# JohannesBuchner/UltraNest

Measured on AMD Instinct MI355X. Metric: proposal-points filtered/sec (MLFriends.inside) + region-rebuild ms, N=4000 d=50, higher is better.
Workload: dtype f64; 1 GPU; C5: N=4000 live points, d=50, P=1e6 proposals/step/GPU drawn uniformly inside the wrapping ellipsoid (set E), AffineLayer, 30 bootstraps; one step = MLFriends.inside on a batch resident in HBM; the timed loop visits 3 distinct batches in turn; n_live=4000, d=50, bootstraps=30, parallelism=proposal rows sharded over 1 GPU(s), region replicated

## Files before the change

include/mlfriends_hip.h:

```cpp
#ifndef MLFRIENDS_HIP_H
#define MLFRIENDS_HIP_H

#include <stddef.h>
#include <stdint.h>

#ifdef __cplusplus
extern "C" {
#endif

#define MLF_ABI_VERSION 5

#define MLF_E_BADARG 1
#define MLF_E_DIM 2
#define MLF_E_NODEVICE 3
#define MLF_E_STATE 4

#define MLF_MAX_DIM 1024

int mlf_abi_version(void);
const char *mlf_last_error(void);
int mlf_device_count(int *count);
int mlf_set_device(int device);
int mlf_device_name(char *buf, size_t buflen);
int mlf_synchronize(void);
// ... 254 lines not shown
                           uint64_t seed, uint64_t offset, int slots_per_poll, mlf_usermodel *model, double *out_u,
                           double *out_p, double *out_L, int64_t *out_start, double *out_tleft, double *out_tright,
                           int32_t *out_taken, int32_t *out_taken_it, int32_t *out_iters, double *out_widths,
                           double *counts, uint64_t *next_offset);

int mlf_region_time_inside_dev(mlf_region *r, const double *d_pts, size_t np, uint8_t *d_mask,
                               void *stream, int reps, float *ms_total, float *ms_scan);

int mlf_region_inside_dev_timed(mlf_region *r, const double *d_pts, size_t np, uint8_t *d_mask,
                                void *stream);
int mlf_region_timing_collect(mlf_region *r, int *ncalls, double *ms_prep, double *ms_scan,
                              double *ms_rest);
int mlf_region_timing_filter_launches(mlf_region *r, int *nlaunches, double *ms_total);
int mlf_region_timing_filter_launch_ms(mlf_region *r, double *ms, int cap, int *nlaunches);
int mlf_region_filter_info(mlf_region *r, size_t np, int *active, int *kdim, int *ntiles32);
int mlf_comm_unique_id(char *id_out, size_t len );
int mlf_comm_init_rank(const char *id, size_t len, int nranks, int rank);
int mlf_comm_init(int ndev);
int mlf_allreduce_max(double *values, size_t count);
int mlf_comm_destroy(void);

int mlf_region_debug_stats(mlf_region *r, unsigned long long *out, int cap);
int mlf_region_debug_fused_stamps(mlf_region *r, int block, unsigned long long *out, int cap);
int mlf_bench_fp64_valu(double *tflops);

#ifdef __cplusplus
}
#endif
#endif
```

ultranest_amd/_lib.py:

```python
import ctypes
import os

import numpy as np

_HERE = os.path.dirname(os.path.abspath(__file__))
LIB_PATH = os.path.join(_HERE, "libmlfriends_hip.so")

ABI_VERSION = 5

_c_double_p = ctypes.c_void_p
_sz = ctypes.c_size_t
_dbl = ctypes.c_double
_int = ctypes.c_int
_vp = ctypes.c_void_p

SIGNATURES = {
    "mlf_abi_version": [],
    "mlf_last_error": [],
    "mlf_device_count": [_vp],
    "mlf_set_device": [_int],
    "mlf_device_name": [_vp, _sz],
    "mlf_synchronize": [],
    "mlf_set_option": [ctypes.c_char_p, ctypes.c_longlong],
    "mlf_get_option": [ctypes.c_char_p, _vp],
# ... 68 lines not shown
    "mlf_walkers_update_live": [_vp, _vp, _sz, _vp, _vp],
    "mlf_walkers_step_dev": [_vp, _dbl, _dbl, _int, _dbl, ctypes.c_uint64, ctypes.c_uint64, _int, _dbl, _dbl, _int, _vp, _dbl,
                             _vp, _vp],
    "mlf_walkers_step_graph": [_vp, _dbl, _dbl, _int, _dbl, ctypes.c_uint64, ctypes.c_uint64, _int, _dbl, _dbl, _int, _vp, _dbl,
                               _vp, _vp],
    "mlf_walkers_rounds_dev": [_vp, _dbl, _dbl, _int, _dbl, ctypes.c_uint64, ctypes.c_uint64, _int, _dbl, _dbl, _int, _vp, _dbl,
                               _int, _vp, _vp, _vp, _vp],
    "mlf_walkers_export": [_vp, _vp, _vp, _vp, _vp, _vp, _vp, _vp, _vp, _vp],
    "mlf_host_changed_rows": [_vp, _vp, _sz, _sz, _vp, _sz, _vp],
    "mlf_host_draw_selection": [_vp, _vp, _sz, _sz, _vp],
    "mlf_counter_create": [_vp, _sz, _sz, _vp, _int, _int],
    "mlf_counter_destroy": [_vp],
    "mlf_counter_reset": [_vp],
    "mlf_counter_passing_node": [_vp, ctypes.c_int64, _dbl, _sz, _vp, _vp, _vp, _sz, _vp, _vp],
    "mlf_counter_state": [_vp, _vp, _vp, _vp, _vp, _vp, _vp, _sz, _vp],
    "mlf_region_inside_dev_timed": [_vp, _vp, _sz, _vp, _vp],
    "mlf_region_timing_collect": [_vp, _vp, _vp, _vp, _vp],
    "mlf_region_timing_filter_launches": [_vp, _vp, _vp],
    "mlf_region_timing_filter_launch_ms": [_vp, _vp, ctypes.c_int, _vp],
    "mlf_region_filter_info": [_vp, _sz, _vp, _vp, _vp],
    "mlf_bench_fp64_valu": [_vp],
    "mlf_region_debug_stats": [_vp, _vp, _int],
    "mlf_region_debug_fused_stamps": [_vp, _int, _vp, _int],
    "mlf_comm_unique_id": [_vp, _sz],
    "mlf_comm_init_rank": [_vp, _sz, _int, _int],
    "mlf_comm_init": [_int],
    "mlf_allreduce_max": [_vp, _sz],
    "mlf_comm_destroy": [],
    "mlf_usermodel_compile": [ctypes.c_char_p, ctypes.c_char_p, _int, _vp, _sz, _vp, _vp, _sz],
    "mlf_usermodel_create": [_vp, _sz, _sz, _int, _vp, _sz, _vp],
    "mlf_usermodel_destroy": [_vp],
    "mlf_usermodel_eval": [_vp, _vp, _sz, _vp, _vp],
    "mlf_usermodel_eval_dev": [_vp, _vp, _sz, _vp, _vp, _vp, _vp],
    "mlf_region_refill_user": [_vp, _int, _sz, ctypes.c_uint64, ctypes.c_uint64, _dbl, _vp, _vp, _vp, _vp, _sz, _vp, _vp, _vp],
    "mlf_region_set_tregion": [_vp, _vp, _vp, _vp, _dbl],
    "mlf_region_set_tregion_center": [_vp, _vp],
    "mlf_region_clear_tregion": [_vp],
    "mlf_region_set_tregion_wide": [_vp, _sz, _vp, _vp, _vp, _dbl],
    "mlf_usermodel_compile_variant": [ctypes.c_char_p, ctypes.c_char_p, _int, _int, _vp, _sz, _vp, _vp, _sz],
    "mlf_usermodel_compile_sums": [ctypes.c_char_p, ctypes.c_char_p, _int, _int, _int, _vp, _sz, _vp, _vp, _sz],
    "mlf_usermodel_create_variant": [_vp, _sz, _sz, _int, _int, _vp, _sz, _vp],
    "mlf_usermodel_create_sum": [_vp, _sz, _sz, _int, _int, _sz, _vp, _sz, _vp],
    "mlf_usermodel_create_derived": [_vp, _sz, _sz, _sz, _vp, _sz, _vp],
    "mlf_usermodel_derive": [_vp, _vp, _sz, _vp],
    "mlf_usermodel_derive_dev": [_vp, _vp, _sz, _vp, _vp],
    "mlf_usermodel_derive_lds_bytes": [_sz, _sz],
# ... 146 lines not shown
```

ultranest_amd/csrc/mlf_debug.hip:

```cpp
#include <hip/hip_runtime.h>

#include <atomic>
#include <vector>

#include "../../include/mlfriends_hip.h"
#include "mlf_host.hpp"
#include "mlf_sample.hpp"

using namespace mlf;

extern "C" {

int mlf_debug_forget_grants(unsigned long long *grants_so_far) {
  if (grants_so_far) *grants_so_far = g_grant_calls.load(std::memory_order_relaxed);
  g_grant_epoch.fetch_add(1u, std::memory_order_acq_rel);
  return 0;
}

int mlf_debug_philox(uint64_t seed, unsigned stream, size_t nblocks, uint32_t *out) {
  if (!out) return fail_arg(MLF_E_BADARG, "null pointer");
  if (nblocks == 0) return 0;
  if (int rc = ensure_ctx()) return rc;
  Ctx &c = g_ctx;
  CK(c.out.reserve(nblocks * 4 * sizeof(unsigned)));
// ... 73 lines not shown
  *nlaunches = n;
  return 0;
}

int mlf_region_filter_info(mlf_region *r, size_t np, int *active, int *kdim, int *ntiles32) {
  if (!r || !active || !kdim || !ntiles32) return fail_arg(MLF_E_BADARG, "null pointer");
  *active = (r->ready && r->use_scan && plan_batch(r->filter, r, BATCH_INSIDE, (long long)np, r->r2).filter) ? 1 : 0;
  *kdim = r->filter.ks * 16;
  *ntiles32 = r->filter.ntiles32;
  return 0;
}

int mlf_region_debug_fused_stamps(mlf_region *r, int block, unsigned long long *out, int cap) {
  if (!r) return fail_arg(MLF_E_BADARG, "null region");
  FilterCtx &f = r->filter;
  if (out && cap > 0) {
    for (int i = 0; i < cap; ++i) out[i] = 0ull;
    if (f.fstamps.p && f.stamp_block >= 0) {
      CK(hipStreamSynchronize(g_ctx.stream));
      CK(hipMemcpy(out, f.fstamps.p, (size_t)(cap < 16 ? cap : 16) * sizeof(unsigned long long), hipMemcpyDeviceToHost));
    }
  }
  f.stamp_block = block;
  return 0;
}

int mlf_region_debug_stats(mlf_region *r, unsigned long long *out, int cap) {
  if (!r || !out || cap < 6) return fail_arg(MLF_E_BADARG, "bad argument");
  FilterCtx &f = r->filter;
  for (int i = 0; i < cap; ++i) out[i] = 0;
  CK(hipDeviceSynchronize());
  if (f.misc.p) {
    unsigned m[8];
    CK(hipMemcpy(m, f.misc.p, sizeof m, hipMemcpyDeviceToHost));
    out[0] = m[4];
  }
  if (f.segcnt.p && f.segcnt.cap >= sizeof(unsigned)) {
    const size_t n = (size_t)f.last.nsegs;
    std::vector<unsigned> c(n);
    if (n) CK(hipMemcpy(c.data(), f.segcnt.p, n * sizeof(unsigned), hipMemcpyDeviceToHost));
    unsigned long long sum = 0, mx = 0;
    for (unsigned v : c) {
      sum += v;
      mx = v > mx ? v : mx;
    }
    out[2] = sum;
// ... 83 lines not shown
```

ultranest_amd/csrc/mlf_filter.hpp:

```cpp
#pragma once
#include "mlf_common.hpp"
#include "mlf_prep4.hpp"

#define MLF_FILTER_MAXD 128

constexpr int kFilterMaxSplit = 16;

namespace mlf {

struct FilterArgs {
  const void *refF;
  const void *qF;
  const float *tlo, *thi;
  int ntiles32;
  long long ngroups;
  long long nq;
  int *best;
  unsigned long long *list;
  unsigned seg_cap;
  unsigned *seg_count;
  unsigned *counters;
  int tile0, tile1;
  const int *qmap;
  const unsigned *ngroups_dev;
// ... 88 lines not shown
};
#define MLF_FOR_EACH_DP_MID(X)                                                                \
  X(2) X(4) X(6) X(8) X(10) X(12) X(14) X(16) X(18) X(20) X(22) X(24) X(26) X(28) X(30) X(32) \
  X(36) X(40) X(44) X(48) X(50) X(52) X(56)
bool mid_usable(int dp);
int mid_range_quads(long long ngroups, int ntiles32);
hipError_t launch_inside_mid(const MidArgs &a, int ny, hipStream_t s);

struct FusedArgs {
  Prep4Args p;
  const void *refF;
  int ntiles32;
  int tile0, tile1;
  void *cq;
  float *ctlo, *cthi;
  int *cmap, *cmin;
  unsigned *ccount;
  unsigned ccap;
  unsigned long long *stamps;
  unsigned stamp_block;
  unsigned variant;
};
bool fused_usable(int dp);
hipError_t launch_prep_sweep(const FusedArgs &a, hipStream_t s, int waves = 8);

void launch_phase_finish(void *cq, float *ctlo, float *cthi, int *cmap, unsigned *ccount, unsigned *ngroups_dst,
                         int ks, hipStream_t s);

struct RecheckArgs {
  const unsigned long long *list;
  unsigned seg_cap;
  const unsigned *seg_count;
  const double *refR;
  int n, d, dp;
  const double *q;
  long long ldq, ldk, nq;
  double r2;
  int *best;
};

void launch_ref_stats(const double *refR, int n, int d, int dp, double *stats, double *scratch, hipStream_t s,
                      unsigned long long *keys = nullptr);
void launch_quant_refs(const double *refR, int n, int npad32, int d, int dp, int ks,
                       const double *stats, void *refF, hipStream_t s, void *refFm = nullptr, const int *perm = nullptr,
                       double *rows_out = nullptr, int nrows_out = 0);
void launch_ref_rank(const unsigned long long *keys, int n, int *perm, hipStream_t s);
void launch_quant_queries(const double *q, long long ldq, long long nq, long long nqpad, int d_src, int d, int ks,
// ... 16 lines not shown
```

ultranest_amd/csrc/mlf_fused.hip:

```cpp
#include "mlf_filter.hpp"
#include "mlf_dpp_dev.hpp"
#include "mlf_filter_dev.hpp"
#include "mlf_prep4.hpp"

#include <math.h>

namespace mlf {

typedef float float16v __attribute__((ext_vector_type(16)));
typedef _Float16 half2v __attribute__((ext_vector_type(2)));
typedef _Float16 half8v __attribute__((ext_vector_type(8)));
typedef float float2v __attribute__((ext_vector_type(2)));
typedef unsigned uint4v __attribute__((ext_vector_type(4)));

#ifndef MLF_OPERAND_STEPS
#define MLF_OPERAND_STEPS 4
#endif
namespace {

template <int DP, int NW = 8>
struct F4 {
  static constexpr int NS = (DP + 15) / 16;
  static constexpr int KS = (DP + 6 + 15) / 16;
  static constexpr int NT = (KS + 1) / 2;
  static constexpr int NE = (DP + 31) / 32;
  static constexpr int KMIN = DP <= 32 ? DP - 1 : (DP == 50 ? 49 : DP - 3);
  static constexpr int NLT = NS + (NE > 1 ? NS - 2 : 0);
  static constexpr int NPC = (DP + 3) / 4;
  static constexpr size_t r16(size_t x) { return (x + 15) / 16 * 16; }
  static constexpr size_t WAVE = NW == 8 ? r16((size_t)NPC * 1024 + 512) : r16((size_t)32 * DP * 8);
  static constexpr size_t FRAG = (size_t)(2 * NT * NS + 2 * NLT) * 1024 + (size_t)(32 * NE + 32 * NT) * 4 + (size_t)(16 * NS) * 8;
  static constexpr size_t LDS = r16(FRAG) + NW * WAVE + 64 + (NW == 8 ? 0 : 128);
};

template <int NS, int NE, int NT>
struct F4Steps {
  static constexpr int NYE = NS + (NE > 1 ? NS - 2 : 0);
  static constexpr int N = NYE + NT * NS;
  static constexpr int ye_find(int i, bool want_t) {
    int c = 0;
    for (int s = 0; s < NS; ++s)
      for (int t = 0; t < NE; ++t)
        if (s >= 2 * t) {
          if (c == i) return want_t ? t : s;
          ++c;
        }
    return 0;
  }
  static constexpr bool is_t(int i) { return i >= NYE; }
  static constexpr int tile(int i) { return i < NYE ? ye_find(i, true) : (i - NYE) % NT; }
  static constexpr int kstep(int i) { return i < NYE ? ye_find(i, false) : (i - NYE) / NT; }
  static constexpr int fragment(int i) { return i < NYE ? (tile(i) ? NS : 0) + kstep(i) - 2 * tile(i) : tile(i) * NS + kstep(i); }
  static constexpr bool first_of_chain(int i) { return i >= NYE && kstep(i) == 0; }
};

// ... 9 lines not shown
__device__ __forceinline__ float half_sum(float v) { return half_sum32(v); }
__device__ __forceinline__ int min3i(int a, int b, int c) {
  const int m = a < b ? a : b;
  return m < c ? m : c;
}
constexpr int kPosInf = 0x7f800000;
__device__ __forceinline__ int tree_min(const float16v &c, int run) {
  const int m0 = min3i(__float_as_int(c[0]), __float_as_int(c[1]), __float_as_int(c[2]));
  const int m1 = min3i(__float_as_int(c[3]), __float_as_int(c[4]), __float_as_int(c[5]));
  const int m2 = min3i(__float_as_int(c[6]), __float_as_int(c[7]), __float_as_int(c[8]));
  const int m3 = min3i(__float_as_int(c[9]), __float_as_int(c[10]), __float_as_int(c[11]));
  const int m4 = min3i(__float_as_int(c[12]), __float_as_int(c[13]), __float_as_int(c[14]));
  return min3i(min3i(m0, m1, m2), min3i(m3, m4, __float_as_int(c[15])), run);
}
template <int I, int NM, int NV>
__device__ __forceinline__ void pin_step() {
  if constexpr (I < NM) {
    __builtin_amdgcn_sched_group_barrier(0x008, 1, 0);
    __builtin_amdgcn_sched_group_barrier(0x002, (NV * (I + 1)) / NM - (NV * I) / NM, 0);
    pin_step<I + 1, NM, NV>();
  }
}

}

template <int DP, int NW, bool SQ>
__global__ __launch_bounds__(64 * NW, NW == 8 ? 1 : 2) void k_prep_sweep(FusedArgs a) {
  using C = F4<DP, NW>;
  constexpr int NS = C::NS, NT = C::NT, NE = C::NE, KS = C::KS, QW = 4;
  extern __shared__ __attribute__((aligned(16))) unsigned char ldsf[];
  const uint4 *Th = reinterpret_cast<const uint4 *>(ldsf);
  const uint4 *Tl = Th + NT * NS * 64;
  const uint4 *Lh = Tl + NT * NS * 64;
  const uint4 *Ll = Lh + C::NLT * 64;
  float *y0l = reinterpret_cast<float *>(const_cast<uint4 *>(Ll + C::NLT * 64));
  float *csl = y0l + 32 * NE;
  double *ctrl = reinterpret_cast<double *>(csl + 32 * NT);
  const int tid = threadIdx.x, lane = tid & 63;
  const int wv = __builtin_amdgcn_readfirstlane(tid >> 6);
  const int p32 = lane & 31, h = lane >> 5;
  unsigned char *area = ldsf + C::r16(C::FRAG) + (size_t)wv * C::WAVE;
  double *xs = reinterpret_cast<double *>(area);
  const int d = a.p.d;
  constexpr float up = 1.0f + 0x1p-18f, dn = 1.0f - 0x1p-18f;
  unsigned *wg_keep = reinterpret_cast<unsigned *>(ldsf + C::r16(C::FRAG) + NW * C::WAVE);
  unsigned &wg_base = wg_keep[8];
  const bool stamp_on = a.stamps != nullptr && blockIdx.x == a.stamp_block && wv == 0;
  auto stamp = [&](int k) __attribute__((always_inline)) {
    if (stamp_on) {
      const unsigned long long t = __builtin_readcyclecounter();
      if (lane == 0) a.stamps[k] = t;
    }
  };
  stamp(0);

  const double sigma = a.p.stats[0];
  const bool sig_ok = sigma >= 0x1p-60 && sigma <= 0x1p60;
  const float sig_f = sig_ok ? (float)sigma : 1.0f;
  if (blockIdx.x == 0 && tid == 0 && a.p.counters) {
    a.p.counters[0] = 0;
    a.p.counters[1] = 0;
  }
  if (!(a.variant & 1u)) {
    uint4 *dst = reinterpret_cast<uint4 *>(ldsf);
    const uint4 *srcT = reinterpret_cast<const uint4 *>(a.p.TtF);
    const uint4 *srcL = reinterpret_cast<const uint4 *>(a.p.LtF);
    for (int e = tid; e < 2 * NT * NS * 64; e += 64 * NW) dst[e] = srcT[e];
    if constexpr (!SQ)
      for (int e = tid; e < 2 * C::NLT * 64; e += 64 * NW) dst[2 * NT * NS * 64 + e] = srcL[e];
  } else {
    typedef __attribute__((address_space(1))) const void gp_t;
    typedef __attribute__((address_space(3))) void lp_t;
    constexpr int NPT = 2 * NT * NS, NPL = SQ ? 0 : 2 * C::NLT;
    const unsigned char *srcT = reinterpret_cast<const unsigned char *>(a.p.TtF);
    const unsigned char *srcL = reinterpret_cast<const unsigned char *>(a.p.LtF);
#pragma unroll
    for (int i = 0; i < (NPT + NPL + NW - 1) / NW; ++i) {
      const int pc = wv + NW * i;
      if (pc < NPT)
        __builtin_amdgcn_global_load_lds((gp_t *)(srcT + (size_t)pc * 1024 + lane * 16), (lp_t *)(ldsf + (size_t)pc * 1024), 16, 0, 0);
      else if (pc < NPT + NPL)
        __builtin_amdgcn_global_load_lds((gp_t *)(srcL + (size_t)(pc - NPT) * 1024 + lane * 16), (lp_t *)(ldsf + (size_t)pc * 1024), 16, 0, 0);
    }
  }
  static_assert(32 * NE <= 64 * NW && 32 * NT <= 64 * NW && 16 * NS <= 64 * NW, "one thread per constant");
  if constexpr (!SQ)
    if (tid < 32 * NE) y0l[tid] = a.p.y0[tid];
  if (tid < 32 * NT) {
    const int col = f4_column(tid >> 5, tid & 31);
    csl[tid] = col < DP ? 2.0f * (float)(sigma * a.p.stats[8 + col]) : 0.0f;
  }
  if (tid < 16 * NS) ctrl[tid] = tid < d ? (double)a.p.c.s_x * a.p.lay_ctr[tid] : 0.0;

  const long long np = a.p.np;
  const long long ngroups = (np + 31) / 32;
  const long long set = (long long)blockIdx.x * NW + wv;
  const long long g0 = set * QW;
  const long long total = np * (long long)d;
  typedef __attribute__((address_space(1))) const void gptr_t;
  typedef __attribute__((address_space(3))) void lptr_t;
  const int units = 16 * d, nfull = units >> 6, rem = units & 63;
  auto fetch_group = [&](long long grp) __attribute__((always_inline)) {
    if (grp >= ngroups) return;
    const long long base = grp * 32 * (long long)d;
    if (base + 32 * (long long)d <= total) {
      const unsigned char *src = reinterpret_cast<const unsigned char *>(a.p.pts + base) + lane * 16;
      int nf = nfull;
      asm volatile("" : "+s"(nf));
#pragma unroll
      for (int ib = 0; ib < C::NPC; ib += 4) {
        gptr_t *gp = (gptr_t *)(src + ib * 1024);
        lptr_t *lp = (lptr_t *)(area + ib * 1024);
        if (ib < nf) __builtin_amdgcn_global_load_lds(gp, lp, 16, 0, 0);
        if (ib + 1 < C::NPC && ib + 1 < nf) __builtin_amdgcn_global_load_lds(gp, lp, 16, 1024, 0);
        if (ib + 2 < C::NPC && ib + 2 < nf) __builtin_amdgcn_global_load_lds(gp, lp, 16, 2048, 0);
        if (ib + 3 < C::NPC && ib + 3 < nf) __builtin_amdgcn_global_load_lds(gp, lp, 16, 3072, 0);
      }
      if (lane < rem)
        __builtin_amdgcn_global_load_lds((gptr_t *)(src + nf * 1024), (lptr_t *)(area + nf * 1024), 16, 0, 0);
    } else {
#pragma nounroll
      for (int e = lane; e < units; e += 64) {
        const long long g = base + 2 * e;
        double v0 = 0.0, v1 = 0.0;
        if (g < total) v0 = a.p.pts[g];
        if (g + 1 < total) v1 = a.p.pts[g + 1];
        xs[2 * e] = v0;
        xs[2 * e + 1] = v1;
      }
    }
  };
  fetch_group(g0);
  if (a.variant & 1u) asm volatile("s_waitcnt vmcnt(0)" ::: "memory");
  __syncthreads();
  stamp(1);

  const float sqrt_k = __builtin_sqrtf((float)(16 * KS));
  const float namax = (float)a.p.stats[1] * up;
  float cs2 = 0.0f;
  for (int e = 0; e < 32 * NT; ++e) cs2 = __builtin_fmaf(csl[e], csl[e], cs2);
  const float csn = 0.5f * __builtin_sqrtf(cs2) * up;
  const float zeta_scale = sig_f * a.p.c.zt * up;
  const float zeta0 = (a.p.c.g_chain * csn + sig_f * a.p.c.zt_abs) * up + 0x1p-100f;
  const float kappa = -2.0f * sig_f * a.p.c.inv_st_sx;
  const double sr = sigma * sqrt(a.p.r2);
  const float sr_lo = (float)(sr * (1.0 - 0x1p-30)) * dn;
  const float sr_hi = (float)(sr * (1.0 + 0x1p-30)) * up;
  const float inv_sx2 = a.p.c.inv_sx * a.p.c.inv_sx, inv_slsx2 = a.p.c.inv_sl_sx * a.p.c.inv_sl_sx;
  const double sxd = (double)a.p.c.s_x;

  half8v bq[QW][KS];
  float tlo[QW], thi[QW];
  half8v hia[NS], loa[NS];
  float dn2a = 0.0f;
  typedef __attribute__((address_space(3))) const double lds_cdouble;
  lds_cdouble *xrow = (lds_cdouble *)(xs + p32 * d + 8 * h);
  lds_cdouble *crow = (lds_cdouble *)(ctrl + 8 * h);
  asm volatile("" : "+v"(xrow), "+v"(crow));
  auto operands = [&]() __attribute__((always_inline)) {
    float dn2 = 0.0f;
    constexpr int SB = MLF_OPERAND_STEPS;
#pragma unroll
    for (int sb = 0; sb < NS; sb += SB) {
      double xv[SB][8], cv[SB][8];
#pragma unroll
      for (int s = sb; s < sb + SB && s < NS; ++s)
#pragma unroll
        for (int jj = 0; jj < 8; ++jj) {
          if (16 * s + (jj & ~1) >= DP) continue;
          xv[s - sb][jj] = xrow[16 * s + jj];
// ... 27 lines not shown
          }
          float x32[2];
#pragma unroll
          for (int e = 0; e < 2; ++e) {
            const int jj = 2 * j2 + e;
            const int k = 16 * s + 8 * h + jj;
            const bool ok = 16 * s + 8 + jj < C::KMIN || k < d;
            const double x = __builtin_fma(xv[s - sb][jj], sxd, -cv[s - sb][jj]);
            x32[e] = ok ? (float)x : 0.0f;
            dn2 = __builtin_fmaf(x32[e], x32[e], dn2);
          }
          const half2v hp = __builtin_convertvector((float2v){x32[0], x32[1]}, half2v);
          const float2v res = {x32[0] - (float)hp[0], x32[1] - (float)hp[1]};
          const half2v lp = __builtin_convertvector(res, half2v);
          hia[s][2 * j2] = hp[0];
          hia[s][2 * j2 + 1] = hp[1];
          loa[s][2 * j2] = lp[0];
          loa[s][2 * j2 + 1] = lp[1];
        }
      }
    }
    return dn2;
  };
  auto frag = [&](const uint4 *base, int idx) __attribute__((always_inline)) {
    union { uint4 u; half8v h8; } cv;
    cv.u = base[idx * 64 + lane];
    return cv.h8;
  };
  if (g0 < ngroups) {
    asm volatile("s_waitcnt vmcnt(0)" ::: "memory");
    __builtin_amdgcn_wave_barrier();
    stamp(2);
    dn2a = operands();
    asm volatile("s_waitcnt lgkmcnt(0)" ::: "memory");
    __builtin_amdgcn_wave_barrier();
    fetch_group(g0 + 1);
  }
#pragma unroll
  for (int g = 0; g < QW; ++g) {
    const long long grp = g0 + g;
    unsigned pk[KS * 4];
#pragma unroll
    for (int i = 0; i < KS * 4; ++i) pk[i] = 0u;
    float lo_f = -1.0f, hi_f = -1.0f;
    if (grp < ngroups) {
      const long long p = grp * 32 + p32;
      const bool live = p < np;
      unsigned char pre = 1;
// ... 127 lines not shown
      sp[2].v = (half2v){p2, p3};
#pragma unroll
      for (int q = 0; q < 3; ++q) {
        const int c = DP + 2 * q;
        if (h == ((c >> 3) & 1)) pk[4 * (c >> 4) + ((c & 7) >> 1)] = sp[q].u;
      }
      if (rt != 1) {
#pragma unroll
        for (int i = 0; i < KS * 4; ++i) pk[i] = 0u;
      }
      if (__any(rt == 2) && lane == 0) *a.p.scan_flag = 1u;
      if (live && h == 0) {
        a.p.route[p] = (uint8_t)rt;
        a.p.best[p] = kNone;
      }
      stamp(3 + 2 * g);
      if (g + 1 < QW && grp + 1 < ngroups) {
        asm volatile("s_waitcnt vmcnt(0)" ::: "memory");
        __builtin_amdgcn_wave_barrier();
        stamp(4 + 2 * g);
        dn2a = operands();
        asm volatile("s_waitcnt lgkmcnt(0)" ::: "memory");
        __builtin_amdgcn_wave_barrier();
        if (g + 2 < QW) fetch_group(grp + 2);
      }
    }
#pragma unroll
    for (int s = 0; s < KS; ++s) {
      union { uint4v u; half8v h8; } cv;
      cv.u = (uint4v){pk[4 * s], pk[4 * s + 1], pk[4 * s + 2], pk[4 * s + 3]};
      bq[g][s] = cv.h8;
    }
    tlo[g] = low_half32(lo_f);
    thi[g] = low_half32(hi_f);
  }

  int run[QW];
#pragma unroll
  for (int g = 0; g < QW; ++g) run[g] = kPosInf;
  bool any_valid = false;
#pragma unroll
  for (int g = 0; g < QW; ++g) any_valid = any_valid || thi[g] > 0.0f;
  if (g0 < ngroups && __any(any_valid)) {
    const int ntl = a.tile1 - a.tile0;
    const int tstart = a.tile0 + (int)((set * 37) % ntl);
    constexpr int kTileBytes = KS * 1024;
    const __amdgpu_buffer_rsrc_t rsrc =
// ... 58 lines not shown
  unsigned keepm[QW];
  int qmn[QW];
  unsigned total_keep = 0u;
#pragma unroll
  for (int g = 0; g < QW; ++g) {
    keepm[g] = 0u;
    qmn[g] = kPosInf;
    if (g0 + g >= ngroups) continue;
    const long long qi = (g0 + g) * 32 + p32;
    const int m = half_min32(run[g]);
    const float mf = __int_as_float(m);
    const bool valid = qi < np && thi[g] > 0.0f;
    const bool hit = valid && mf <= tlo[g];
    if (lane < 32 && hit) a.p.best[qi] = 0;
    keepm[g] = (unsigned)__ballot(valid && !hit);
    qmn[g] = m;
    total_keep += (unsigned)__popc(keepm[g]);
  }
  if (lane == 0) wg_keep[wv] = total_keep;
  __syncthreads();
  if (tid == 0) {
    unsigned all = 0u;
    for (int w = 0; w < NW; ++w) all += wg_keep[w];
    wg_base = all ? atomicAdd(a.ccount, all) : 0u;
  }
  __syncthreads();
  if (total_keep != 0u) {
    unsigned base = wg_base;
    for (int w = 0; w < wv; ++w) base += wg_keep[w];
    base = (unsigned)__builtin_amdgcn_readfirstlane((int)base);
    uint4 *dst = reinterpret_cast<uint4 *>(a.cq);
    const unsigned row = (unsigned)p32;
#pragma unroll
    for (int g = 0; g < QW; ++g) {
      if ((keepm[g] >> row) & 1u) {
        const unsigned rank = base + (unsigned)__popc(keepm[g] & ((1u << row) - 1u));
        const size_t gd = rank >> 5;
        const unsigned rd = (rank & 31u) + (unsigned)(lane & 32);
        if (rank < a.ccap) {
#pragma unroll
          for (int s = 0; s < KS; ++s) {
            union { half8v h8; uint4 u; } cv;
            cv.h8 = bq[g][s];
            dst[(gd * KS + s) * 64 + rd] = cv.u;
          }
        }
        if (lane < 32 && rank < a.ccap) {
          a.ctlo[rank] = tlo[g];
          a.cthi[rank] = thi[g];
          a.cmap[rank] = (int)((g0 + g) * 32 + p32);
          a.cmin[rank] = qmn[g];
        }
      }
      base += (unsigned)__popc(keepm[g]);
    }
  }
  stamp(12);
}

bool fused_usable(int dp) { return dp >= 2 && dp <= 56 && (dp & 1) == 0; }

template <int D, int NW, bool SQ>
static hipError_t launch_prep_sweep_t(const FusedArgs &a, long long nsets, hipStream_t s) {
  constexpr size_t lds = F4<D, NW>::LDS;
  static_assert(lds <= 160 * 1024 - 64, "LDS budget");
  static DeviceGrant grant;
  if (hipError_t e = grant.ensure([] {
        return hipFuncSetAttribute(reinterpret_cast<const void *>(&k_prep_sweep<D, NW, SQ>), hipFuncAttributeMaxDynamicSharedMemorySize, (int)lds);
      }))
    return e;
  if (a.p.ks != F4<D, NW>::KS) return hipErrorInvalidValue;
  const dim3 grid((unsigned)((nsets + NW - 1) / NW));
  hipLaunchKernelGGL((k_prep_sweep<D, NW, SQ>), grid, dim3(64 * NW), lds, s, a);
  return hipGetLastError();
}

hipError_t launch_prep_sweep(const FusedArgs &a, hipStream_t s, int waves) {
  if (a.p.np <= 0) return hipSuccess;
  const long long ngroups = (a.p.np + 31) / 32;
  const long long nsets = (ngroups + 3) / 4;
  const bool sq = (a.variant & 2u) != 0u;
  switch (a.p.dp) {
#define X(D)                                                                                  \
  case D:                                                                                     \
    if constexpr (2 * F4<D, 4>::LDS <= 160 * 1024) {                                          \
      if (waves == 4) return sq ? launch_prep_sweep_t<D, 4, true>(a, nsets, s) : launch_prep_sweep_t<D, 4, false>(a, nsets, s); \
    }                                                                                         \
    return sq ? launch_prep_sweep_t<D, 8, true>(a, nsets, s) : launch_prep_sweep_t<D, 8, false>(a, nsets, s);
    MLF_FOR_EACH_DP_MID(X)
#undef X
    default:
      return hipErrorInvalidValue;
  }
}

}
```

ultranest_amd/csrc/mlf_host.hpp:

```cpp
#pragma once
#include <cmath>
#include <vector>

#include "mlf_ctx.hpp"
#include "mlf_filter.hpp"
#include "mlf_misc.hpp"
#include "mlf_small.hpp"
#include "mlf_wide_filter.hpp"

namespace mlf {

constexpr unsigned kFilterSegCap = 2048;
constexpr long long kFilterMinQueriesDefault = 257;

enum Opt : int {
  OPT_FILTER,
  OPT_FIRST_RANGE_PCT,
  OPT_SPLIT_WAVES,
  OPT_NARROW_TAIL,
  OPT_SMALL_PATH,
  OPT_FUSED_PREP,
  OPT_PHASE_MIN_QUERIES,
  OPT_PHASES,
  OPT_TIME_LAUNCHES,
// ... 52 lines not shown
  unsigned fused_variant = 0;
  int fused_waves = 4;
  long long nsegs = 0;
  long long seg_room = 0;
};

struct FilterCtx {
  bool refs_ready = false;
  bool refs_dirty = false;
  bool usable = false;
  int ks = 0, ntiles32 = 0;
  bool wide = false;
  double sigma = 1.0, amax = 0.0;
  DevBuf stats, statscratch, refF, qF, tlo, thi, route, best, counters, list, segcnt, gate2;
  DevBuf refFm, refRm, okeys, operm;
  bool ordered = false;
  int order_n = -1;
  DevBuf pqF[2], ptlo[2], pthi[2], pmap[2], png, pmin, pmin2;
  DevBuf mid_rec, mid_meta, mid_arrive;
  bool mid_dirty = false;
  DevBuf wstatscratch;
  DevBuf fstamps;
  int stamp_block = -1;
  bool png_dirty = false;
  DevBuf ell_list, misc;
  unsigned batch_parity = 0;
  BatchPlan last;
  BatchPlan last_min;
  std::vector<hipEvent_t> kev;
  size_t kev_used = 0;
  OptOverrides ov;
  void release() {
    DevBuf *b[] = {&stats, &statscratch, &refF, &qF, &tlo, &thi, &route, &best, &counters, &list, &segcnt, &gate2, &refFm, &refRm, &okeys, &operm,
                   &pqF[0], &pqF[1], &ptlo[0], &ptlo[1], &pthi[0], &pthi[1], &pmap[0], &pmap[1], &png, &pmin, &pmin2, &mid_rec, &mid_meta, &mid_arrive,
                   &ell_list, &misc, &fstamps, &wstatscratch};
    for (DevBuf *x : b) x->release();
    refs_ready = usable = ordered = wide = false;
    order_n = -1;
  }
};

inline long long opt(const FilterCtx &f, int id) { return f.ov.set[id] ? f.ov.v[id] : g_opt[id]; }

struct Ctx {
  bool ready = false;
  int device = 0;
// ... 148 lines not shown
```

ultranest_amd/csrc/mlf_route.hip:

```cpp
#include <hip/hip_runtime.h>

#include <algorithm>

#include "../../include/mlfriends_hip.h"
#include "mlf_host.hpp"
#include "mlf_prep3.hpp"
#include "mlf_prep64.hpp"

namespace mlf {

int filter_prepare_refs(FilterCtx &f, const double *refR, int n, int d, int dp, hipStream_t s,
                        bool host_sync, bool mask_mode) {
  f.refs_ready = false;
  f.wide = false;
  const int ks = (dp + 6 + 15) / 16;
  const bool wide = ks > 9;
  if ((wide && (!mask_mode || ks > kWideFilterMaxKs)) || n < 1 ||
      (long long)round_up(n, 32) / 32 * ks * 1024 >= (1ll << 31)) {
    f.usable = false;
    return 0;
  }
  f.ks = ks;
  const int npad32 = round_up(n, 32);
  f.ntiles32 = npad32 / 32;
// ... 260 lines not shown
  m.ccount = f.png.as<unsigned>() + 2;
  m.last = 0;
  if (p.defer) {
    FusedArgs fu{};
    fu.p = xs.prep;
    fu.refF = b.opF();
    fu.ntiles32 = f.ntiles32;
    fu.tile0 = 0;
    fu.tile1 = p.cut[0];
    fu.cq = m.cq;
    fu.ctlo = m.ctlo;
    fu.cthi = m.cthi;
    fu.cmap = m.cmap;
    fu.cmin = m.cmin;
    fu.ccount = m.ccount;
    fu.ccap = m.ccap;
    if (f.stamp_block >= 0 && f.stamp_block < 1000000) {
      CK(f.fstamps.reserve(16 * sizeof(unsigned long long)));
      fu.stamps = f.fstamps.as<unsigned long long>();
      fu.stamp_block = (unsigned)f.stamp_block;
    }
    fu.variant = p.fused_variant;
    if (fu.variant & 2u) fu.p.c = xs.same;
    if (int rc = timed_launch(b, [&] { return launch_prep_sweep(fu, b.s, p.fused_waves); })) return rc;
  } else if (int rc = timed_launch(b, [&] { return launch_sweep_min(f.ks, filter_groups_per_wave(f.ks, 0), m, b.s); })) {
    return rc;
  }
  const int usrc = min3 ? 0 : 1;
  m.tile0 = p.cut[0];
  m.tile1 = min3 ? p.cut[1] : f.ntiles32;
  m.qF = f.pqF[0].p;
  m.tlo = f.ptlo[0].as<float>();
  m.thi = f.pthi[0].as<float>();
  m.qmap = f.pmap[0].as<int>();
  m.qmin = f.pmin.as<int>();
  m.nslots_dev = f.png.as<unsigned>() + 2;
  m.cq = f.pqF[1].p;
  m.ctlo = f.ptlo[1].as<float>();
  m.cthi = f.pthi[1].as<float>();
  m.cmap = f.pmap[1].as<int>();
  m.cmin = min3 ? f.pmin2.as<int>() : nullptr;
  m.ccount = f.png.as<unsigned>() + 3;
  m.last = min3 ? 0 : 1;
  auto sweep_stamps = [&](int which) -> int {
    m.stamps = nullptr;
    if (f.stamp_block >= which * 1000000 && f.stamp_block < (which + 1) * 1000000) {
      CK(f.fstamps.reserve(16 * sizeof(unsigned long long)));
// ... 290 lines not shown
```

ultranest_amd/kernels.py:

```python
import ctypes

import numpy as np

from . import _lib
from ._lib import check, f64, ptr

int_dtype = np.int64


def find_nearby(apts, bpts, radiussq, nnearby):
    apts, bpts = f64(apts), f64(bpts)
    if apts.ndim != 2 or bpts.ndim != 2:
        raise ValueError("apts and bpts must be 2-d")
    nb = bpts.shape[0]
    d = bpts.shape[1] if nb else apts.shape[1]
    if nb and apts.shape[0] and apts.shape[1] != bpts.shape[1]:
        raise ValueError("dimensionality mismatch")
    if nnearby.dtype != int_dtype or nnearby.ndim != 1 or len(nnearby) != nb:
        raise ValueError("nnearby must be an int64 vector of len(bpts)")
    out = nnearby if nnearby.flags.c_contiguous else np.empty(nb, dtype=int_dtype)
    check(_lib.lib().mlf_find_nearby(ptr(apts), apts.shape[0], ptr(bpts), nb, d, float(radiussq), ptr(out)))
    if out is not nnearby:
        nnearby[:] = out

# ... 375 lines not shown
        check(_lib.lib().mlf_region_filter_info(self._h, int(npts), ctypes.byref(act), ctypes.byref(k), ctypes.byref(t)))
        return bool(act.value), k.value, t.value

    def debug_stats(self):
        out = np.zeros(19, dtype=np.uint64)
        check(_lib.lib().mlf_region_debug_stats(self._h, ptr(out), 19))
        keys = ("ellipsoid_band", "exact_scan_queries", "uncertain_pairs", "largest_segment", "segments", "second_range_groups",
                "uncertain_queries", "third_range_groups")
        stats = {k: int(v) for k, v in zip(keys, out[:8]) if k}
        stats["range_cuts"] = [int(out[16]), int(out[17])]
        stats["same_quadratic_form"] = int(out[18])
        if out[8]:
            st = out[8:16].astype(np.int64)
            stats["uncertain_stage_cycles"] = [int((st[i + 1] - st[i]) & 0xffffffff) for i in range(6) if st[i + 1]]
            stats["stamp7"] = int(st[7])
        return stats

    def fused_stamps(self, block):
        out = np.zeros(16, dtype=np.uint64)
        check(_lib.lib().mlf_region_debug_fused_stamps(self._h, -1 if block is None else int(block), ptr(out), 16))
        st = out[:16].astype(np.int64)
        return [int(x - st[0]) if x else None for x in st] if st[0] else None

    def time_inside_dev(self, d_pts, npts, d_mask, stream=0, reps=3):
        tot, scan = ctypes.c_float(0), ctypes.c_float(0)
        check(_lib.lib().mlf_region_time_inside_dev(self._h, ctypes.c_void_p(d_pts), npts, ctypes.c_void_p(d_mask),
                                                    ctypes.c_void_p(stream), int(reps), ctypes.byref(tot),
                                                    ctypes.byref(scan)))
        return tot.value, scan.value


def bench_fp64_valu():
    t = ctypes.c_double(0)
    check(_lib.lib().mlf_bench_fp64_valu(ctypes.byref(t)))
    return t.value


def philox_blocks(seed, stream, nblocks):
    out = np.empty((int(nblocks), 4), dtype=np.uint32)
    check(_lib.lib().mlf_debug_philox(ctypes.c_uint64(int(seed)), int(stream), int(nblocks), ptr(out)))
    return out
```

Baseline: 3.020 billion proposals/s.

## Make fused prep-sweep kernel persistent with per-block prologue reuse and next-set prefetch

```diff
diff --git a/include/mlfriends_hip.h b/include/mlfriends_hip.h
--- a/include/mlfriends_hip.h
+++ b/include/mlfriends_hip.h
@@ -300,6 +300,7 @@
 
 int mlf_region_debug_stats(mlf_region *r, unsigned long long *out, int cap);
 int mlf_region_debug_fused_stamps(mlf_region *r, int block, unsigned long long *out, int cap);
+int mlf_region_debug_fused_grid_cap(mlf_region *r, int cap);
 int mlf_bench_fp64_valu(double *tflops);
 
 #ifdef __cplusplus
diff --git a/ultranest_amd/_lib.py b/ultranest_amd/_lib.py
--- a/ultranest_amd/_lib.py
+++ b/ultranest_amd/_lib.py
@@ -114,6 +114,7 @@
     "mlf_bench_fp64_valu": [_vp],
     "mlf_region_debug_stats": [_vp, _vp, _int],
     "mlf_region_debug_fused_stamps": [_vp, _int, _vp, _int],
+    "mlf_region_debug_fused_grid_cap": [_vp, _int],
     "mlf_comm_unique_id": [_vp, _sz],
     "mlf_comm_init_rank": [_vp, _sz, _int, _int],
     "mlf_comm_init": [_int],
diff --git a/ultranest_amd/csrc/mlf_debug.hip b/ultranest_amd/csrc/mlf_debug.hip
--- a/ultranest_amd/csrc/mlf_debug.hip
+++ b/ultranest_amd/csrc/mlf_debug.hip
@@ -119,6 +119,13 @@
     }
   }
   f.stamp_block = block;
+  return 0;
+}
+
+int mlf_region_debug_fused_grid_cap(mlf_region *r, int cap) {
+  if (!r) return fail_arg(MLF_E_BADARG, "null region");
+  if (cap < 0) return fail_arg(MLF_E_BADARG, "negative grid cap");
+  r->filter.fused_grid_cap = cap;
   return 0;
 }
 
diff --git a/ultranest_amd/csrc/mlf_filter.hpp b/ultranest_amd/csrc/mlf_filter.hpp
--- a/ultranest_amd/csrc/mlf_filter.hpp
+++ b/ultranest_amd/csrc/mlf_filter.hpp
@@ -134,7 +134,7 @@
   unsigned variant;
 };
 bool fused_usable(int dp);
-hipError_t launch_prep_sweep(const FusedArgs &a, hipStream_t s, int waves = 8);
+hipError_t launch_prep_sweep(const FusedArgs &a, hipStream_t s, int waves = 8, int grid_cap = 0);
 
 void launch_phase_finish(void *cq, float *ctlo, float *cthi, int *cmap, unsigned *ccount, unsigned *ngroups_dst,
                          int ks, hipStream_t s);
diff --git a/ultranest_amd/csrc/mlf_fused.hip b/ultranest_amd/csrc/mlf_fused.hip
--- a/ultranest_amd/csrc/mlf_fused.hip
+++ b/ultranest_amd/csrc/mlf_fused.hip
@@ -13,6 +13,11 @@
 typedef float float2v __attribute__((ext_vector_type(2)));
 typedef unsigned uint4v __attribute__((ext_vector_type(4)));
 
+#ifdef MLF_FUSED_BODY_INLINE
+#define MLF_FUSED_BODY_ATTR __forceinline__
+#else
+#define MLF_FUSED_BODY_ATTR __attribute__((noinline))
+#endif
 #ifndef MLF_OPERAND_STEPS
 #define MLF_OPERAND_STEPS 4
 #endif
@@ -30,7 +35,7 @@
   static constexpr size_t r16(size_t x) { return (x + 15) / 16 * 16; }
   static constexpr size_t WAVE = NW == 8 ? r16((size_t)NPC * 1024 + 512) : r16((size_t)32 * DP * 8);
   static constexpr size_t FRAG = (size_t)(2 * NT * NS + 2 * NLT) * 1024 + (size_t)(32 * NE + 32 * NT) * 4 + (size_t)(16 * NS) * 8;
-  static constexpr size_t LDS = r16(FRAG) + NW * WAVE + 64 + (NW == 8 ? 0 : 128);
+  static constexpr size_t LDS = r16(FRAG) + NW * WAVE + 192;
 };
 
 template <int NS, int NE, int NT>
@@ -86,130 +91,103 @@
   }
 }
 
+__device__ __forceinline__ int uni(int v) { return __builtin_amdgcn_readfirstlane(v); }
+__device__ __forceinline__ long long uni(long long v) {
+  const unsigned lo = (unsigned)__builtin_amdgcn_readfirstlane((int)(unsigned)v);
+  const unsigned hi = (unsigned)__builtin_amdgcn_readfirstlane((int)(unsigned)((unsigned long long)v >> 32));
+  return (long long)(((unsigned long long)hi << 32) | lo);
+}
+template <class T>
+using lds_t = __attribute__((address_space(3))) T;
+typedef __attribute__((address_space(4))) const FusedArgs kargs_t;
+
+template <int NPC>
+__device__ __forceinline__ void fetch_group_rows(const double *pts, long long np, int d, long long grp, lds_t<unsigned char> *area, int lane) {
+  typedef __attribute__((address_space(1))) const void gptr_t;
+  typedef __attribute__((address_space(3))) void lptr_t;
+  const long long ngroups = (np + 31) / 32, total = np * (long long)d;
+  if (grp >= ngroups) return;
+  const int units = 16 * d, nfull = units >> 6, rem = units & 63;
+  const long long base = grp * 32 * (long long)d;
+  if (base + 32 * (long long)d <= total) {
+    const unsigned char *src = reinterpret_cast<const unsigned char *>(pts + base) + lane * 16;
+    int nf = nfull;
+    asm volatile("" : "+s"(nf));
+#pragma unroll
+    for (int ib = 0; ib < NPC; ib += 4) {
+      gptr_t *gp = (gptr_t *)(src + ib * 1024);
+      lptr_t *lp = (lptr_t *)(area + ib * 1024);
+      if (ib < nf) __builtin_amdgcn_global_load_lds(gp, lp, 16, 0, 0);
+      if (ib + 1 < NPC && ib + 1 < nf) __builtin_amdgcn_global_load_lds(gp, lp, 16, 1024, 0);
+      if (ib + 2 < NPC && ib + 2 < nf) __builtin_amdgcn_global_load_lds(gp, lp, 16, 2048, 0);
+      if (ib + 3 < NPC && ib + 3 < nf) __builtin_amdgcn_global_load_lds(gp, lp, 16, 3072, 0);
+    }
+    if (lane < rem)
+      __builtin_amdgcn_global_load_lds((gptr_t *)(src + nf * 1024), (lptr_t *)(area + nf * 1024), 16, 0, 0);
+  } else {
+    lds_t<double> *xs = reinterpret_cast<lds_t<double> *>(area);
+#pragma nounroll
+    for (int e = lane; e < units; e += 64) {
+      const long long g = base + 2 * e;
+      double v0 = 0.0, v1 = 0.0;
+      if (g < total) v0 = pts[g];
+      if (g + 1 < total) v1 = pts[g + 1];
+      xs[2 * e] = v0;
+      xs[2 * e + 1] = v1;
+    }
+  }
+}
+
 }
 
 template <int DP, int NW, bool SQ>
-__global__ __launch_bounds__(64 * NW, NW == 8 ? 1 : 2) void k_prep_sweep(FusedArgs a) {
+__device__ MLF_FUSED_BODY_ATTR void prep_sweep_set(const FusedArgs *ka_, unsigned lds_, int blk_, int nblk_, int stride_, int pass_) {
   using C = F4<DP, NW>;
   constexpr int NS = C::NS, NT = C::NT, NE = C::NE, KS = C::KS, QW = 4;
-  extern __shared__ __attribute__((aligned(16))) unsigned char ldsf[];
-  const uint4 *Th = reinterpret_cast<const uint4 *>(ldsf);
-  const uint4 *Tl = Th + NT * NS * 64;
-  const uint4 *Lh = Tl + NT * NS * 64;
-  const uint4 *Ll = Lh + C::NLT * 64;
-  float *y0l = reinterpret_cast<float *>(const_cast<uint4 *>(Ll + C::NLT * 64));
-  float *csl = y0l + 32 * NE;
-  double *ctrl = reinterpret_cast<double *>(csl + 32 * NT);
+  kargs_t &a = *(kargs_t *)(uintptr_t)uni((long long)reinterpret_cast<uintptr_t>(ka_));
+  lds_t<unsigned char> *ldsf = (lds_t<unsigned char> *)(uintptr_t)(unsigned)uni((int)lds_);
+  const int blk = uni(blk_), nblk = uni(nblk_), stride = uni(stride_), pass = uni(pass_);
+  const lds_t<uint4v> *Th = reinterpret_cast<const lds_t<uint4v> *>(ldsf);
+  const lds_t<uint4v> *Tl = Th + NT * NS * 64;
+  const lds_t<uint4v> *Lh = Tl + NT * NS * 64;
+  const lds_t<uint4v> *Ll = Lh + C::NLT * 64;
+  const lds_t<float> *y0l = reinterpret_cast<const lds_t<float> *>(Ll + C::NLT * 64);
+  const lds_t<float> *csl = y0l + 32 * NE;
+  const lds_t<double> *ctrl = reinterpret_cast<const lds_t<double> *>(csl + 32 * NT);
   const int tid = threadIdx.x, lane = tid & 63;
   const int wv = __builtin_amdgcn_readfirstlane(tid >> 6);
   const int p32 = lane & 31, h = lane >> 5;
-  unsigned char *area = ldsf + C::r16(C::FRAG) + (size_t)wv * C::WAVE;
-  double *xs = reinterpret_cast<double *>(area);
+  lds_t<unsigned char> *area = ldsf + C::r16(C::FRAG) + (size_t)wv * C::WAVE;
+  lds_t<double> *xs = reinterpret_cast<lds_t<double> *>(area);
   const int d = a.p.d;
   constexpr float up = 1.0f + 0x1p-18f, dn = 1.0f - 0x1p-18f;
-  unsigned *wg_keep = reinterpret_cast<unsigned *>(ldsf + C::r16(C::FRAG) + NW * C::WAVE);
-  unsigned &wg_base = wg_keep[8];
-  const bool stamp_on = a.stamps != nullptr && blockIdx.x == a.stamp_block && wv == 0;
+  lds_t<unsigned> *tail = reinterpret_cast<lds_t<unsigned> *>(ldsf + C::r16(C::FRAG) + NW * C::WAVE);
+  lds_t<unsigned> *wg_keep = tail + 16 * (pass & 1);
+  const lds_t<unsigned> *rcu = tail + 32;
+  const lds_t<float> *rc = reinterpret_cast<const lds_t<float> *>(rcu);
+  const bool stamp_wave = a.stamps != nullptr && blockIdx.x == a.stamp_block && wv == 0;
+  const bool stamp_on = stamp_wave && pass == 0;
   auto stamp = [&](int k) __attribute__((always_inline)) {
     if (stamp_on) {
       const unsigned long long t = __builtin_readcyclecounter();
       if (lane == 0) a.stamps[k] = t;
     }
   };
-  stamp(0);
-
-  const double sigma = a.p.stats[0];
-  const bool sig_ok = sigma >= 0x1p-60 && sigma <= 0x1p60;
-  const float sig_f = sig_ok ? (float)sigma : 1.0f;
-  if (blockIdx.x == 0 && tid == 0 && a.p.counters) {
-    a.p.counters[0] = 0;
-    a.p.counters[1] = 0;
-  }
-  if (!(a.variant & 1u)) {
-    uint4 *dst = reinterpret_cast<uint4 *>(ldsf);
-    const uint4 *srcT = reinterpret_cast<const uint4 *>(a.p.TtF);
-    const uint4 *srcL = reinterpret_cast<const uint4 *>(a.p.LtF);
-    for (int e = tid; e < 2 * NT * NS * 64; e += 64 * NW) dst[e] = srcT[e];
-    if constexpr (!SQ)
-      for (int e = tid; e < 2 * C::NLT * 64; e += 64 * NW) dst[2 * NT * NS * 64 + e] = srcL[e];
-  } else {
-    typedef __attribute__((address_space(1))) const void gp_t;
-    typedef __attribute__((address_space(3))) void lp_t;
-    constexpr int NPT = 2 * NT * NS, NPL = SQ ? 0 : 2 * C::NLT;
-    const unsigned char *srcT = reinterpret_cast<const unsigned char *>(a.p.TtF);
-    const unsigned char *srcL = reinterpret_cast<const unsigned char *>(a.p.LtF);
-#pragma unroll
-    for (int i = 0; i < (NPT + NPL + NW - 1) / NW; ++i) {
-      const int pc = wv + NW * i;
-      if (pc < NPT)
-        __builtin_amdgcn_global_load_lds((gp_t *)(srcT + (size_t)pc * 1024 + lane * 16), (lp_t *)(ldsf + (size_t)pc * 1024), 16, 0, 0);
-      else if (pc < NPT + NPL)
-        __builtin_amdgcn_global_load_lds((gp_t *)(srcL + (size_t)(pc - NPT) * 1024 + lane * 16), (lp_t *)(ldsf + (size_t)pc * 1024), 16, 0, 0);
-    }
-  }
-  static_assert(32 * NE <= 64 * NW && 32 * NT <= 64 * NW && 16 * NS <= 64 * NW, "one thread per constant");
-  if constexpr (!SQ)
-    if (tid < 32 * NE) y0l[tid] = a.p.y0[tid];
-  if (tid < 32 * NT) {
-    const int col = f4_column(tid >> 5, tid & 31);
-    csl[tid] = col < DP ? 2.0f * (float)(sigma * a.p.stats[8 + col]) : 0.0f;
-  }
-  if (tid < 16 * NS) ctrl[tid] = tid < d ? (double)a.p.c.s_x * a.p.lay_ctr[tid] : 0.0;
-
+  if (stamp_wave && pass == 1) {
+    const unsigned long long t = __builtin_readcyclecounter();
+    if (lane == 0) a.stamps[13] = t;
+  }
   const long long np = a.p.np;
   const long long ngroups = (np + 31) / 32;
-  const long long set = (long long)blockIdx.x * NW + wv;
+  const long long set = (long long)blk * NW + wv;
   const long long g0 = set * QW;
-  const long long total = np * (long long)d;
-  typedef __attribute__((address_space(1))) const void gptr_t;
-  typedef __attribute__((address_space(3))) void lptr_t;
-  const int units = 16 * d, nfull = units >> 6, rem = units & 63;
-  auto fetch_group = [&](long long grp) __attribute__((always_inline)) {
-    if (grp >= ngroups) return;
-    const long long base = grp * 32 * (long long)d;
-    if (base + 32 * (long long)d <= total) {
-      const unsigned char *src = reinterpret_cast<const unsigned char *>(a.p.pts + base) + lane * 16;
-      int nf = nfull;
-      asm volatile("" : "+s"(nf));
-#pragma unroll
-      for (int ib = 0; ib < C::NPC; ib += 4) {
-        gptr_t *gp = (gptr_t *)(src + ib * 1024);
-        lptr_t *lp = (lptr_t *)(area + ib * 1024);
-        if (ib < nf) __builtin_amdgcn_global_load_lds(gp, lp, 16, 0, 0);
-        if (ib + 1 < C::NPC && ib + 1 < nf) __builtin_amdgcn_global_load_lds(gp, lp, 16, 1024, 0);
-        if (ib + 2 < C::NPC && ib + 2 < nf) __builtin_amdgcn_global_load_lds(gp, lp, 16, 2048, 0);
-        if (ib + 3 < C::NPC && ib + 3 < nf) __builtin_amdgcn_global_load_lds(gp, lp, 16, 3072, 0);
-      }
-      if (lane < rem)
-        __builtin_amdgcn_global_load_lds((gptr_t *)(src + nf * 1024), (lptr_t *)(area + nf * 1024), 16, 0, 0);
-    } else {
-#pragma nounroll
-      for (int e = lane; e < units; e += 64) {
-        const long long g = base + 2 * e;
-        double v0 = 0.0, v1 = 0.0;
-        if (g < total) v0 = a.p.pts[g];
-        if (g + 1 < total) v1 = a.p.pts[g + 1];
-        xs[2 * e] = v0;
-        xs[2 * e + 1] = v1;
-      }
-    }
-  };
-  fetch_group(g0);
-  if (a.variant & 1u) asm volatile("s_waitcnt vmcnt(0)" ::: "memory");
-  __syncthreads();
-  stamp(1);
+  const bool has_next = blk + stride < nblk;
+  const long long next_g0 = ((long long)(blk + stride) * NW + wv) * QW;
+  auto fetch_group = [&](long long grp) __attribute__((always_inline)) { fetch_group_rows<C::NPC>(a.p.pts, np, d, grp, area, lane); };
 
   const float sqrt_k = __builtin_sqrtf((float)(16 * KS));
-  const float namax = (float)a.p.stats[1] * up;
-  float cs2 = 0.0f;
-  for (int e = 0; e < 32 * NT; ++e) cs2 = __builtin_fmaf(csl[e], csl[e], cs2);
-  const float csn = 0.5f * __builtin_sqrtf(cs2) * up;
-  const float zeta_scale = sig_f * a.p.c.zt * up;
-  const float zeta0 = (a.p.c.g_chain * csn + sig_f * a.p.c.zt_abs) * up + 0x1p-100f;
-  const float kappa = -2.0f * sig_f * a.p.c.inv_st_sx;
-  const double sr = sigma * sqrt(a.p.r2);
-  const float sr_lo = (float)(sr * (1.0 - 0x1p-30)) * dn;
-  const float sr_hi = (float)(sr * (1.0 + 0x1p-30)) * up;
+  const bool sig_ok = rcu[0] != 0u;
+  const float namax = rc[2], zeta_scale = rc[3], zeta0 = rc[4], kappa = rc[5], sr_lo = rc[6], sr_hi = rc[7];
   const float inv_sx2 = a.p.c.inv_sx * a.p.c.inv_sx, inv_slsx2 = a.p.c.inv_sl_sx * a.p.c.inv_sl_sx;
   const double sxd = (double)a.p.c.s_x;
 
@@ -283,8 +261,8 @@
     }
     return dn2;
   };
-  auto frag = [&](const uint4 *base, int idx) __attribute__((always_inline)) {
-    union { uint4 u; half8v h8; } cv;
+  auto frag = [&](const lds_t<uint4v> *base, int idx) __attribute__((always_inline)) {
+    union { uint4v u; half8v h8; } cv;
     cv.u = base[idx * 64 + lane];
     return cv.h8;
   };
@@ -458,7 +436,10 @@
         dn2a = operands();
         asm volatile("s_waitcnt lgkmcnt(0)" ::: "memory");
         __builtin_amdgcn_wave_barrier();
-        if (g + 2 < QW) fetch_group(grp + 2);
+        if (g + 2 < QW)
+          fetch_group(grp + 2);
+        else if (has_next)
+          fetch_group(next_g0);
       }
     }
 #pragma unroll
@@ -563,11 +544,11 @@
   if (tid == 0) {
     unsigned all = 0u;
     for (int w = 0; w < NW; ++w) all += wg_keep[w];
-    wg_base = all ? atomicAdd(a.ccount, all) : 0u;
+    wg_keep[8] = all ? atomicAdd(a.ccount, all) : 0u;
   }
   __syncthreads();
   if (total_keep != 0u) {
-    unsigned base = wg_base;
+    unsigned base = wg_keep[8];
     for (int w = 0; w < wv; ++w) base += wg_keep[w];
     base = (unsigned)__builtin_amdgcn_readfirstlane((int)base);
     uint4 *dst = reinterpret_cast<uint4 *>(a.cq);
@@ -599,10 +580,115 @@
   stamp(12);
 }
 
+template <int DP, int NW, bool SQ>
+__global__ __launch_bounds__(64 * NW, NW == 8 ? 1 : 2) void k_prep_sweep(FusedArgs a) {
+  using C = F4<DP, NW>;
+  constexpr int NS = C::NS, NT = C::NT, NE = C::NE;
+  extern __shared__ __attribute__((aligned(16))) unsigned char ldsf[];
+  const uint4 *Th = reinterpret_cast<const uint4 *>(ldsf);
+  const uint4 *Tl = Th + NT * NS * 64;
+  const uint4 *Lh = Tl + NT * NS * 64;
+  const uint4 *Ll = Lh + C::NLT * 64;
+  float *y0l = reinterpret_cast<float *>(const_cast<uint4 *>(Ll + C::NLT * 64));
+  float *csl = y0l + 32 * NE;
+  double *ctrl = reinterpret_cast<double *>(csl + 32 * NT);
+  const int tid = threadIdx.x, lane = tid & 63;
+  const int wv = __builtin_amdgcn_readfirstlane(tid >> 6);
+  const int d = a.p.d;
+  constexpr float up = 1.0f + 0x1p-18f, dn = 1.0f - 0x1p-18f;
+  const bool stamp_on = a.stamps != nullptr && blockIdx.x == a.stamp_block && wv == 0;
+  auto stamp = [&](int k) __attribute__((always_inline)) {
+    if (stamp_on) {
+      const unsigned long long t = __builtin_readcyclecounter();
+      if (lane == 0) a.stamps[k] = t;
+    }
+  };
+  stamp(0);
+
+  const double sigma = a.p.stats[0];
+  const bool sig_ok = sigma >= 0x1p-60 && sigma <= 0x1p60;
+  const float sig_f = sig_ok ? (float)sigma : 1.0f;
+  if (blockIdx.x == 0 && tid == 0 && a.p.counters) {
+    a.p.counters[0] = 0;
+    a.p.counters[1] = 0;
+  }
+  if (!(a.variant & 1u)) {
+    uint4 *dst = reinterpret_cast<uint4 *>(ldsf);
+    const uint4 *srcT = reinterpret_cast<const uint4 *>(a.p.TtF);
+    const uint4 *srcL = reinterpret_cast<const uint4 *>(a.p.LtF);
+    for (int e = tid; e < 2 * NT * NS * 64; e += 64 * NW) dst[e] = srcT[e];
+    if constexpr (!SQ)
+      for (int e = tid; e < 2 * C::NLT * 64; e += 64 * NW) dst[2 * NT * NS * 64 + e] = srcL[e];
+  } else {
+    typedef __attribute__((address_space(1))) const void gp_t;
+    typedef __attribute__((address_space(3))) void lp_t;
+    constexpr int NPT = 2 * NT * NS, NPL = SQ ? 0 : 2 * C::NLT;
+    const unsigned char *srcT = reinterpret_cast<const unsigned char *>(a.p.TtF);
+    const unsigned char *srcL = reinterpret_cast<const unsigned char *>(a.p.LtF);
+#pragma unroll
+    for (int i = 0; i < (NPT + NPL + NW - 1) / NW; ++i) {
+      const int pc = wv + NW * i;
+      if (pc < NPT)
+        __builtin_amdgcn_global_load_lds((gp_t *)(srcT + (size_t)pc * 1024 + lane * 16), (lp_t *)(ldsf + (size_t)pc * 1024), 16, 0, 0);
+      else if (pc < NPT + NPL)
+        __builtin_amdgcn_global_load_lds((gp_t *)(srcL + (size_t)(pc - NPT) * 1024 + lane * 16), (lp_t *)(ldsf + (size_t)pc * 1024), 16, 0, 0);
+    }
+  }
+  static_assert(32 * NE <= 64 * NW && 32 * NT <= 64 * NW && 16 * NS <= 64 * NW, "one thread per constant");
+  if constexpr (!SQ)
+    if (tid < 32 * NE) y0l[tid] = a.p.y0[tid];
+  if (tid < 32 * NT) {
+    const int col = f4_column(tid >> 5, tid & 31);
+    csl[tid] = col < DP ? 2.0f * (float)(sigma * a.p.stats[8 + col]) : 0.0f;
+  }
+  if (tid < 16 * NS) ctrl[tid] = tid < d ? (double)a.p.c.s_x * a.p.lay_ctr[tid] : 0.0;
+
+  if (wv == 0) {
+    float cs2 = 0.0f;
+#pragma unroll
+    for (int e = 0; e < 32 * NT; ++e) {
+      const int col = f4_column(e >> 5, e & 31);
+      const float cse = col < DP ? 2.0f * (float)(sigma * a.p.stats[8 + (col < DP ? col : 0)]) : 0.0f;
+      cs2 = __builtin_fmaf(cse, cse, cs2);
+    }
+    const float csn = 0.5f * __builtin_sqrtf(cs2) * up;
+    const double sr = sigma * sqrt(a.p.r2);
+    if (lane == 0) {
+      unsigned *rcu = reinterpret_cast<unsigned *>(ldsf + C::r16(C::FRAG) + NW * C::WAVE) + 32;
+      float *rc = reinterpret_cast<float *>(rcu);
+      rcu[0] = sig_ok ? 1u : 0u;
+      rc[1] = sig_f;
+      rc[2] = (float)a.p.stats[1] * up;
+      rc[3] = sig_f * a.p.c.zt * up;
+      rc[4] = (a.p.c.g_chain * csn + sig_f * a.p.c.zt_abs) * up + 0x1p-100f;
+      rc[5] = -2.0f * sig_f * a.p.c.inv_st_sx;
+      rc[6] = (float)(sr * (1.0 - 0x1p-30)) * dn;
+      rc[7] = (float)(sr * (1.0 + 0x1p-30)) * up;
+    }
+  }
+  const long long nblk = (((a.p.np + 31) / 32 + 3) / 4 + NW - 1) / NW;
+  fetch_group_rows<C::NPC>(a.p.pts, a.p.np, d, ((long long)blockIdx.x * NW + wv) * 4,
+                           (lds_t<unsigned char> *)(ldsf + C::r16(C::FRAG) + (size_t)wv * C::WAVE), lane);
+  if (a.variant & 1u) asm volatile("s_waitcnt vmcnt(0)" ::: "memory");
+  __syncthreads();
+  stamp(1);
+
+  const FusedArgs *ka = (const FusedArgs *)__builtin_amdgcn_kernarg_segment_ptr();
+  const unsigned lds0 = (unsigned)(uintptr_t)(lds_t<unsigned char> *)ldsf;
+  int pass = 0;
+#pragma nounroll
+  for (int blk = (int)blockIdx.x; blk < (int)nblk; blk += (int)gridDim.x, ++pass) {
+#ifdef MLF_FUSED_BODY_INLINE
+    asm volatile("" ::: "memory");
+#endif
+    prep_sweep_set<DP, NW, SQ>(ka, lds0, blk, (int)nblk, (int)gridDim.x, pass);
+  }
+}
+
 bool fused_usable(int dp) { return dp >= 2 && dp <= 56 && (dp & 1) == 0; }
 
 template <int D, int NW, bool SQ>
-static hipError_t launch_prep_sweep_t(const FusedArgs &a, long long nsets, hipStream_t s) {
+static hipError_t launch_prep_sweep_t(const FusedArgs &a, long long nsets, hipStream_t s, int grid_cap) {
   constexpr size_t lds = F4<D, NW>::LDS;
   static_assert(lds <= 160 * 1024 - 64, "LDS budget");
   static DeviceGrant grant;
@@ -611,12 +697,22 @@
       }))
     return e;
   if (a.p.ks != F4<D, NW>::KS) return hipErrorInvalidValue;
-  const dim3 grid((unsigned)((nsets + NW - 1) / NW));
+  static int cus = 0;
+  if (cus == 0) {
+    int dev = 0, n = 0;
+    if (hipError_t e = hipGetDevice(&dev)) return e;
+    if (hipError_t e = hipDeviceGetAttribute(&n, hipDeviceAttributeMultiprocessorCount, dev)) return e;
+    cus = n > 0 ? n : 1;
+  }
+  const long long nblk = (nsets + NW - 1) / NW;
+  long long slots = (long long)cus * (NW == 8 ? 1 : 2);
+  if (grid_cap > 0 && grid_cap < slots) slots = grid_cap;
+  const dim3 grid((unsigned)(nblk < slots ? nblk : slots));
   hipLaunchKernelGGL((k_prep_sweep<D, NW, SQ>), grid, dim3(64 * NW), lds, s, a);
   return hipGetLastError();
 }
 
-hipError_t launch_prep_sweep(const FusedArgs &a, hipStream_t s, int waves) {
+hipError_t launch_prep_sweep(const FusedArgs &a, hipStream_t s, int waves, int grid_cap) {
   if (a.p.np <= 0) return hipSuccess;
   const long long ngroups = (a.p.np + 31) / 32;
   const long long nsets = (ngroups + 3) / 4;
@@ -625,9 +721,9 @@
 #define X(D)                                                                                  \
   case D:                                                                                     \
     if constexpr (2 * F4<D, 4>::LDS <= 160 * 1024) {                                          \
-      if (waves == 4) return sq ? launch_prep_sweep_t<D, 4, true>(a, nsets, s) : launch_prep_sweep_t<D, 4, false>(a, nsets, s); \
+      if (waves == 4) return sq ? launch_prep_sweep_t<D, 4, true>(a, nsets, s, grid_cap) : launch_prep_sweep_t<D, 4, false>(a, nsets, s, grid_cap); \
     }                                                                                         \
-    return sq ? launch_prep_sweep_t<D, 8, true>(a, nsets, s) : launch_prep_sweep_t<D, 8, false>(a, nsets, s);
+    return sq ? launch_prep_sweep_t<D, 8, true>(a, nsets, s, grid_cap) : launch_prep_sweep_t<D, 8, false>(a, nsets, s, grid_cap);
     MLF_FOR_EACH_DP_MID(X)
 #undef X
     default:
diff --git a/ultranest_amd/csrc/mlf_host.hpp b/ultranest_amd/csrc/mlf_host.hpp
--- a/ultranest_amd/csrc/mlf_host.hpp
+++ b/ultranest_amd/csrc/mlf_host.hpp
@@ -98,6 +98,7 @@
   DevBuf wstatscratch;
   DevBuf fstamps;
   int stamp_block = -1;
+  int fused_grid_cap = 0;
   bool png_dirty = false;
   DevBuf ell_list, misc;
   unsigned batch_parity = 0;
diff --git a/ultranest_amd/csrc/mlf_route.hip b/ultranest_amd/csrc/mlf_route.hip
--- a/ultranest_amd/csrc/mlf_route.hip
+++ b/ultranest_amd/csrc/mlf_route.hip
@@ -306,7 +306,7 @@
     }
     fu.variant = p.fused_variant;
     if (fu.variant & 2u) fu.p.c = xs.same;
-    if (int rc = timed_launch(b, [&] { return launch_prep_sweep(fu, b.s, p.fused_waves); })) return rc;
+    if (int rc = timed_launch(b, [&] { return launch_prep_sweep(fu, b.s, p.fused_waves, f.fused_grid_cap); })) return rc;
   } else if (int rc = timed_launch(b, [&] { return launch_sweep_min(f.ks, filter_groups_per_wave(f.ks, 0), m, b.s); })) {
     return rc;
   }
diff --git a/ultranest_amd/kernels.py b/ultranest_amd/kernels.py
--- a/ultranest_amd/kernels.py
+++ b/ultranest_amd/kernels.py
@@ -421,6 +421,9 @@
         st = out[:16].astype(np.int64)
         return [int(x - st[0]) if x else None for x in st] if st[0] else None
 
+    def fused_grid_cap(self, cap):
+        check(_lib.lib().mlf_region_debug_fused_grid_cap(self._h, int(cap)))
+
     def time_inside_dev(self, d_pts, npts, d_mask, stream=0, reps=3):
         tot, scan = ctypes.c_float(0), ctypes.c_float(0)
         check(_lib.lib().mlf_region_time_inside_dev(self._h, ctypes.c_void_p(d_pts), npts, ctypes.c_void_p(d_mask),
```

Measured after the change: 2.875 billion proposals/s. 0.952x the previous value.
